# yjtang249/MIPSFusion

Hardware: NVIDIA B200
Metric: map_step_rays_per_s (higher is better)
Workload: dtype f32 (decoder contractions as bf16x3 hi/lo splits on tcgen05, fp32 accumulate; encodings, render, losses, Adam in fp32)

## Files before the change

### include/mipsfusion_b200.h

```cpp
#ifndef MIPSFUSION_B200_H
#define MIPSFUSION_B200_H

#include <stdint.h>

#ifdef __cplusplus
extern "C" {
#endif

#define MF_ABI_VERSION 2
#define MF_MAX_LEVELS 16
#define MF_MLP_PARAMS 36577
#define MF_RAW_DIM 10

#define MF_OK 0
#define MF_ERR_INVALID (-1)
#define MF_ERR_CUDA (-2)
#define MF_ERR_UNSUPPORTED (-3)

typedef struct {
    int32_t n_levels, n_features, log2_hashmap_size, base_resolution;
    float scale[MF_MAX_LEVELS];
    uint32_t resolution[MF_MAX_LEVELS];
    uint32_t size[MF_MAX_LEVELS];
    uint32_t offset[MF_MAX_LEVELS + 1];
// ... 74 lines not shown
int mf_field_query_rays_bwd(const float* rays_o, const float* rays_d, const float* z, const mf_field* field_host,
                            const float* d_raw, const void* feat, float* grad_grid, float* grad_mlp, float* d_rays_o,
                            float* d_rays_d, float* workspace, int64_t R, int S, void* stream);

int mf_render_loss_fwd(const float* raw, const float* z, const float* target_rgb, const float* target_d,
                       const int64_t* counts, const mf_render_cfg* cfg_host, float* out_rgb, float* out_depth,
                       float* out_aux, float* out_weights, int32_t* inds, float* losses, float* scratch,
                       int64_t R, int S, void* stream);
int mf_sample_z_ld(const float* target_d, int ld_d, const float* u, const float* lin_uniform, const float* lin_range,
                   const float* lin_fallback, const mf_render_cfg* cfg_host, float* z, int64_t* counts, int64_t R, void* stream);
int mf_render_loss_fwd_ld(const float* raw, const float* z, const float* target_rgb, int ld_rgb, const float* target_d, int ld_d,
                          const int64_t* counts, const mf_render_cfg* cfg_host, float* out_rgb, float* out_depth,
                          float* out_aux, float* out_weights, int32_t* inds, float* losses, float* scratch,
                          int64_t R, int S, void* stream);
int mf_render_loss_bwd(const float* raw, const float* z, const float* target_rgb, const float* target_d,
                       const int64_t* counts, const float* losses, const mf_render_cfg* cfg_host,
                       const float* g_losses, const float* g_rgb, const float* g_depth, float* d_raw,
                       int64_t R, int S, void* stream);
int mf_render_loss_bwd_scalars(const float* raw, const float* z, const float* target_rgb, int ld_rgb, const float* target_d, int ld_d,
                               const float* losses, const mf_render_cfg* cfg_host, const float* g_rgb_loss, const float* g_depth_loss,
                               const float* g_sdf_loss, const float* g_fs_loss, const float* g_rgb, const float* g_depth,
                               float* d_raw, int64_t R, int S, void* stream);

int mf_adam_step(float* p, float* g, float* m, float* v, int64_t n, double lr, double beta1, double beta2,
                 double eps, double weight_decay, int step, int zero_grad, void* stream);

int mf_adam_step_sharded(const uint64_t* peer_bases, int world, int rank, int64_t off_p, int64_t off_g, int64_t off_g_clear,
                         float* m, float* v, int64_t n, double lr, double beta1, double beta2, double eps,
                         double weight_decay, int step, uint64_t multicast_base, void* stream);
int mf_adam_step_pair(float* p0, float* g0, float* m0, float* v0, int64_t n0, double lr0, double eps0, double wd0,
                      float* p1, float* g1, float* m1, float* v1, int64_t n1, double lr1, double eps1, double wd1,
                      double beta1, double beta2, int step, void* stream);
int mf_adam_step_multi(int n_tensors, float* const* p_host, float* const* g_host, float* const* m_host,
                       float* const* v_host, const int64_t* n_host, double lr, double beta1, double beta2, double eps,
                       double weight_decay, int step, int zero_grad, void* stream);

int mf_containment(const float* dirs_cam, const float* depth, const float* pose_c2w, const float* pts, const float* xyz_min,
                   const float* xyz_max, int k, int64_t n, int cross, uint8_t* mask, int64_t* counts, void* stream);

int mf_sample_pixels_uniform(int img_h, int img_w, int num_h, int num_w, int64_t* rows, int64_t* cols, void* stream);
int64_t mf_topk_workspace_size(int64_t n);
int mf_sample_pixels_topk(const float* depth, const float* keys, int img_h, int img_w, int lattice_h, int lattice_w,
                          int num, int64_t* indices, int64_t* rows, int64_t* cols, void* workspace, void* stream);

int mf_gen_rays(const float* dirs_cam, const float* poses, const int64_t* pose_idx, float* rays_o, float* rays_d,
                int64_t R, int K, void* stream);
// ... 89 lines not shown
```

### mipsfusion_b200/_lib.py

```python
import ctypes as C
import os

import torch

_HERE = os.path.dirname(os.path.abspath(__file__))
LIB_PATH = os.environ.get("MIPSFUSION_B200_LIB") or os.path.join(_HERE, "libmipsfusion_b200.so")
HEADER_PATH = os.path.join(os.path.dirname(_HERE), "include", "mipsfusion_b200.h")

MF_MAX_LEVELS = 16
MF_MLP_PARAMS = 36577
MF_RAW_DIM = 10
MF_MAX_SAMPLES = 128


class GridMeta(C.Structure):
    _fields_ = [("n_levels", C.c_int32), ("n_features", C.c_int32), ("log2_hashmap_size", C.c_int32),
                ("base_resolution", C.c_int32), ("scale", C.c_float * MF_MAX_LEVELS),
                ("resolution", C.c_uint32 * MF_MAX_LEVELS), ("size", C.c_uint32 * MF_MAX_LEVELS),
                ("offset", C.c_uint32 * (MF_MAX_LEVELS + 1)), ("hashed", C.c_uint32 * MF_MAX_LEVELS)]


class Field(C.Structure):
    _fields_ = [("grid", C.c_void_p), ("mlp_prep", C.c_void_p), ("norm_a", C.c_double * 3), ("norm_b", C.c_double * 3),
                ("norm_factor", C.c_double), ("decoder_impl", C.c_int32), ("reserved", C.c_int32), ("meta", GridMeta)]
# ... 36 lines not shown
    "mf_debug_kernel_ms": (_I, [_I, _P]),
    "mf_hashgrid_meta": (_I, [_I, _I, _I, _I, _D, C.POINTER(GridMeta)]),
    "mf_hashgrid_fwd": (_I, [_P, _P, C.POINTER(GridMeta), _P, _P, _L, _P]),
    "mf_hashgrid_bwd": (_I, [_P, _P, _P, C.POINTER(GridMeta), _P, _P, _L, _P]),
    "mf_freq_fwd": (_I, [_P, _P, _I, _I, _L, _P]),
    "mf_freq_bwd": (_I, [_P, _P, _P, _I, _I, _L, _P]),
    "mf_mlp_prep_size": (_L, []),
    "mf_mlp_prepare": (_I, [_P, _P, _P]),
    "mf_mlp_fwd": (_I, [_P, _P, _P, _P, _P, _L, _P]),
    "mf_field_bwd_workspace_size": (_L, [_L, _I]),
    "mf_mlp_grad_workspace_size": (_L, []),
    "mf_mlp_bwd": (_I, [_P, _P, _P, _P, _P, _P, _P, _P, _P, _P, _L, _P]),
    "mf_field_query": (_I, [_P, C.POINTER(Field), _I, _P, _L, _P]),
    "mf_field_query_bwd": (_I, [_P, C.POINTER(Field), _I, _P, _P, _P, _P, _P, _L, _P]),
    "mf_sample_z": (_I, [_P, _P, _P, _P, _P, C.POINTER(RenderCfg), _P, _P, _L, _P]),
    "mf_feat_cache_size": (_L, [_L]),
    "mf_field_query_rays": (_I, [_P, _P, _P, C.POINTER(Field), _P, _P, _L, _I, _P]),
    "mf_field_query_rays_bwd": (_I, [_P, _P, _P, C.POINTER(Field), _P, _P, _P, _P, _P, _P, _P, _L, _I, _P]),
    "mf_render_loss_fwd": (_I, [_P, _P, _P, _P, _P, C.POINTER(RenderCfg), _P, _P, _P, _P, _P, _P, _P, _L, _I, _P]),
    "mf_render_loss_bwd": (_I, [_P, _P, _P, _P, _P, _P, C.POINTER(RenderCfg), _P, _P, _P, _P, _L, _I, _P]),
    "mf_render_loss_bwd_scalars": (_I, [_P, _P, _P, _I, _P, _I, _P, C.POINTER(RenderCfg), _P, _P, _P, _P, _P, _P, _P, _L, _I, _P]),
    "mf_sample_z_ld": (_I, [_P, _I, _P, _P, _P, _P, C.POINTER(RenderCfg), _P, _P, _L, _P]),
    "mf_render_loss_fwd_ld": (_I, [_P, _P, _P, _I, _P, _I, _P, C.POINTER(RenderCfg), _P, _P, _P, _P, _P, _P, _P, _L, _I, _P]),
    "mf_adam_step": (_I, [_P, _P, _P, _P, _L, _D, _D, _D, _D, _D, _I, _I, _P]),
    "mf_adam_step_sharded": (_I, [_P, _I, _I, _L, _L, _L, _P, _P, _L, _D, _D, _D, _D, _D, _I, C.c_uint64, _P]),
    "mf_adam_step_pair": (_I, [_P, _P, _P, _P, _L, _D, _D, _D, _P, _P, _P, _P, _L, _D, _D, _D, _D, _D, _I, _P]),
    "mf_adam_step_multi": (_I, [_I, _P, _P, _P, _P, _P, _D, _D, _D, _D, _D, _I, _I, _P]),
    "mf_sample_pixels_uniform": (_I, [_I, _I, _I, _I, _P, _P, _P]),
    "mf_topk_workspace_size": (_L, [_L]),
    "mf_sample_pixels_topk": (_I, [_P, _P, _I, _I, _I, _I, _I, _P, _P, _P, _P, _P]),
    "mf_gen_rays": (_I, [_P, _P, _P, _P, _P, _L, _I, _P]),
    "mf_kf_store": (_I, [_P, _P, _P, _P, _P, _I, _L, _P, _P]),
    "mf_kf_gather_rays": (_I, [_P, _L, _L, _P, _L, _I, _P, _L, _P, _L, _P, _L, _P, _P, _P, _P]),
    "mf_sample_distinct": (_I, [_L, _L, C.c_uint32, _P, _P]),
    "mf_kf_sample_rays": (_I, [_P, _L, _L, _P, _L, _L, _I, _L, _L, _L, C.c_uint32, _P, _P, _P, _P, _P]),
    "mf_frame_sample_rays": (_I, [_P, _P, _P, _I, _I, _L, C.c_uint32, _P, _P, _P, _P]),
    "mf_gen_rays_packed": (_I, [_P, _P, _P, _P, _P, _P, _P, _L, _I, _P]),
    "mf_gen_rays_bwd": (_I, [_P, _P, _P, _P, _P, _L, _I, _P]),
    "mf_gen_rays_packed_bwd": (_I, [_P, _P, _P, _P, _P, _L, _I, _P]),
    "mf_pose_to_c2w": (_I, [_P, _P, _P]),
    "mf_pose_refine_update": (_I, [_P, _P, _P, _P, _P, _D, _D, _I, _P, _P]),
    "mf_track_handoff": (_I, [_P, _P, _P, _P, _P]),
    "mf_ba_pose_init": (_I, [_P, _P, _I, _P, _P, _P]),
    "mf_ba_pose_update": (_I, [_P, _P, _P, _I, _D, _D, _P, _P]),
    "mf_ro_score": (_I, [_P, _P, _P, _P, _P, _P, C.POINTER(Field), _D, _D, _I, _I, _I, _P, _P, _P, _P, _P]),
    "mf_ro_update": (_I, [_P, _P, _P, _I, _D, _P, _P, _P, _P, _P, _P]),
# ... 77 lines not shown
```

### mipsfusion_b200/csrc/field_kernels.cu

```cuda
#include "field_bwd.cuh"
#include "field_launch.cuh"
#include "field_tc_launch.cuh"
#include "field_tc_bwd.cuh"
#include "field_tc_bwd2.cuh"
#include "field_tc_bwd3.cuh"

__device__ __forceinline__ void mlp_prepare_simt(const float* __restrict__ mlp, float* __restrict__ prep, int i) {
    if (i >= PREP_SIMT_SIZE) return;
    float v = 0.f;
    if (i < MF_MLP_PARAMS) {
        v = mlp[i];
    } else if (i >= PREP_F1) {
        int r;
        if (i < PREP_B1) {
            int off, K, Kreal;
            if (i < PREP_F2) { r = i - PREP_F1; off = OFF_W1; K = D_E; Kreal = D_E; }
            else if (i < PREP_F3) { r = i - PREP_F2; off = OFF_W2; K = D_H; Kreal = D_H; }
            else { r = i - PREP_F3; off = OFF_WS1; K = D_SDF_IN; Kreal = D_SDF_IN; }
            const int k = r >> 7, tx = (r >> 3) & 15, i8 = r & 7;
            const int n = tx + 16 * i8;
            v = (k < Kreal) ? mlp[off + n * K + k] : 0.f;
        } else {
            int off, K, KI;
            if (i < PREP_B2) { r = i - PREP_B1; off = OFF_W1; K = D_E; KI = 4; }
// ... 487 lines not shown
    if (N >= (int64_t)1 << 31) { mf_set_error("backward: more than 2^31 points"); return MF_ERR_INVALID; }
    const int64_t nb = act_blocks(N);
    int* idx = reinterpret_cast<int*>(scratch);
    uint32_t* flags = reinterpret_cast<uint32_t*>(idx + N);
    int* blk_cnt = reinterpret_cast<int*>(flags + nb * 32);
    int* count = blk_cnt + nb;
    active_count_kernel<<<(unsigned)nb, ACT_BLK, 0, st>>>(d_raw, N, flags, blk_cnt);
    MF_LAUNCH_CHECK();
    active_fill_kernel<<<(unsigned)nb, ACT_BLK, 0, st>>>(flags, blk_cnt, idx, count);
    MF_LAUNCH_CHECK();
    am->idx = idx; am->count = count;
    return MF_OK;
}

static inline int64_t cta_scratch_words() { return (int64_t)mf_sm_count_cached() * b2::SCR_CTA_WORDS; }

MF_API int64_t mf_field_bwd_workspace_size(int64_t n_points, int want_point_grads) {
    if (n_points < 0) n_points = 0;
    return mf_mlp_grad_workspace_size() + (want_point_grads ? 3 * n_points : 0) + act_scratch_words(n_points) + cta_scratch_words();
}

template <class Src>
static int launch_field_bwd(const FieldDev& d, const Src& src, const float* d_raw, float* grad_grid, float* grad_mlp,
                            float* d_pts, float* workspace, float* scratch, int64_t N, cudaStream_t st) {
    ActiveMap am{nullptr, nullptr};
    int rc0 = compact_active_points(d_raw, N, scratch, &am, st); if (rc0) return rc0;
    if (d_pts) MF_CUDA(cudaMemsetAsync(d_pts, 0, (size_t)N * 3 * sizeof(float), st));
    const bool params = grad_grid != nullptr;
    if (!params && !d_pts) {
        mf_set_error("backward without parameter gradients needs a ray / point gradient output");
        return MF_ERR_INVALID;
    }
    if (!params && d.impl == 1) {
        const int grid = persistent_grid(N, 1);
        int rc = set_smem(field_bwd_dx_kernel<Src>, SMEM_BWD); if (rc) return rc;
        field_bwd_dx_kernel<Src><<<grid, NT, SMEM_BWD, st>>>(d, src, d_raw, d_pts, N, am);
        MF_LAUNCH_CHECK();
        return MF_OK;
    }
    if (d.impl != 1) {
        const int64_t tiles = (N + TC_TP - 1) / TC_TP;
        const int64_t cap = mf_sm_count_cached();
        const int grid = (int)(tiles < cap ? (tiles > 0 ? tiles : 1) : cap);
        mf_ktimer_begin(1, st);
        if (!params) {
            int rc = set_smem(field_bwd_tc_kernel<Src, true, false>, SMEM_TC_BWD); if (rc) return rc;
            field_bwd_tc_kernel<Src, true, false><<<grid, TC_NT, SMEM_TC_BWD, st>>>(d, src, d_raw, nullptr, nullptr, d_pts, N, am, mf_tc_error_flag(), mf_tc_profile_buffer());
            mf_ktimer_end(1, st);
            MF_LAUNCH_CHECK();
// ... 83 lines not shown
MF_API int mf_field_query_rays_bwd(const float* rays_o, const float* rays_d, const float* z, const mf_field* field,
                                   const float* d_raw, const void* feat, float* grad_grid, float* grad_mlp, float* d_rays_o,
                                   float* d_rays_d, float* workspace, int64_t R, int S, void* stream) {
    MF_CHECK_ARG(R >= 0 && S > 0);
    if (R == 0) return MF_OK;
    MF_CHECK_ARG(rays_o && rays_d && z && d_raw && workspace);
    MF_CHECK_ARG((grad_grid == nullptr) == (grad_mlp == nullptr));
    MF_CHECK_ARG(((uintptr_t)grad_grid & 15) == 0);
    MF_CHECK_ARG((d_rays_o == nullptr) == (d_rays_d == nullptr));
    FieldDev d; int rc = mf_field_to_dev(field, &d); if (rc) return rc;
    d.feat = (uint32_t*)feat;
    SrcRays src{rays_o, rays_d, z, S};
    cudaStream_t st = (cudaStream_t)stream;
    float* d_pts = d_rays_o ? workspace + mf_mlp_grad_workspace_size() : nullptr;
    float* scratch = workspace + mf_mlp_grad_workspace_size() + (d_rays_o ? 3 * R * S : 0);
    rc = launch_field_bwd(d, src, d_raw, grad_grid, grad_mlp, d_pts, workspace, scratch, R * S, st);
    if (rc) return rc;
    if (d_rays_o) {
        ray_grad_reduce_kernel<<<(unsigned)((R + 7) / 8), 256, 0, st>>>(d_pts, z, d_rays_o, d_rays_d, R, S);
        MF_LAUNCH_CHECK();
    }
    return MF_OK;
}
```

### mipsfusion_b200/csrc/render_kernels.cu

```cuda
#include <limits.h>

#include "mf_common.cuh"

constexpr int MAX_S = 128;

struct RenderCfgDev {
    int n_u, n_r, perturb, rgb_missing_nz;
    float tr;
    float sctr;
    float T;
    float twoT;
    float depth_trunc;
    float emd_w;
    int ld_rgb, ld_d;
};

static RenderCfgDev cfg_to_dev(const mf_render_cfg* c) {
    RenderCfgDev d;
    d.n_u = c->n_samples_d; d.n_r = c->n_range_d; d.perturb = c->perturb; d.rgb_missing_nz = c->rgb_missing_nz;
    d.tr = (float)c->trunc; d.sctr = (float)(c->sc_factor * c->trunc);
    const double T = c->trunc * c->sc_factor;
    d.T = (float)T; d.twoT = (float)(2.0 * T);
    d.depth_trunc = (float)c->depth_trunc; d.emd_w = (float)c->emd_w;
    d.ld_rgb = 3; d.ld_d = 1;
    return d;
}

__global__ void sample_z_kernel(const float* __restrict__ target_d, const float* __restrict__ u,
                                const float* __restrict__ lin_u, const float* __restrict__ lin_r,
                                const float* __restrict__ lin_fb, RenderCfgDev c, float* __restrict__ z,
                                unsigned long long* __restrict__ counts, int64_t R) {
    extern __shared__ float zs[];
    __shared__ int cnt[2];
    const int64_t r = blockIdx.x;
    const int S = c.n_u + c.n_r;
    const bool has_d = target_d != nullptr;
    const float d = has_d ? target_d[r * c.ld_d] : 0.f;
    const bool around = d > 0.f;
    if (threadIdx.x < 2) cnt[threadIdx.x] = 0;
    for (int e = threadIdx.x; e < S; e += blockDim.x) {
        float v; int rank;
        if (e < c.n_u) {
            v = lin_u[e]; rank = e;
            for (int k = 0; k < c.n_r; ++k) {
                const float sv = around ? __fadd_rn(lin_r[k], d) : lin_fb[k];
                rank += (sv < v);
            }
        } else {
            const int k = e - c.n_u;
            v = around ? __fadd_rn(lin_r[k], d) : lin_fb[k];
            rank = k;
            for (int i = 0; i < c.n_u; ++i) rank += (lin_u[i] <= v);
        }
        zs[rank] = v;
    }
    __syncthreads();
    int n_front = 0, n_sdf = 0;
    for (int j = threadIdx.x; j < S; j += blockDim.x) {
        float zj = zs[j];
        if (c.perturb && u) {
            const float lower = (j == 0) ? zs[0] : 0.5f * __fadd_rn(zs[j], zs[j - 1]);
            const float upper = (j == S - 1) ? zs[S - 1] : 0.5f * __fadd_rn(zs[j + 1], zs[j]);
// ... 121 lines not shown
        sdf2 = fmaf(e2, e2, sdf2);
        if (c.emd_w > 0.f) {
            const float* p = raw + (r * S + s) * MF_RAW_DIM + 5;
            const float gt = __fdiv_rn(__fadd_rn(__fsub_rn(d, zz), c.T), c.twoT) * 4.0f;
            float a = 0.f, b = 0.f;
#pragma unroll
            for (int k = 0; k < 5; ++k) { a = fmaf(p[k], (float)(4 - k), a); b = fmaf(fabsf(gt - (float)k), p[k], b); }
            fs1 = fmaf(a, fm, fs1);
            sdf1 = fmaf(b, sm_, sdf1);
        }
    }
    fs2 = warp_sum(fs2); sdf2 = warp_sum(sdf2); fs1 = warp_sum(fs1); sdf1 = warp_sum(sdf1);
    if (lane == 0) {
        float rs = 0.f;
        if (target_rgb)
#pragma unroll
            for (int k = 0; k < 3; ++k) { const float e = rgb[k] * mk - target_rgb[r * c.ld_rgb + k] * mk; rs = fmaf(e, e, rs); }
        float* sc = scratch + r * 8;
        sc[0] = rs; sc[1] = valid ? (depth - d) * (depth - d) : 0.f; sc[2] = valid ? 1.f : 0.f;
        sc[3] = fs2; sc[4] = sdf2; sc[5] = fs1; sc[6] = sdf1; sc[7] = 0.f;
    }
}

__global__ void __launch_bounds__(1024) loss_finalize_kernel(const float* __restrict__ scratch,
                                                             const unsigned long long* __restrict__ counts,
                                                             RenderCfgDev c, float* __restrict__ losses, int64_t R, int S) {
    __shared__ double red[32][8];
    double s[8] = {0, 0, 0, 0, 0, 0, 0, 0};
    const float4* rows = reinterpret_cast<const float4*>(scratch);
    for (int64_t r = threadIdx.x; r < R; r += 1024) {
        const float4 a = rows[2 * r], b = rows[2 * r + 1];
        s[0] += (double)a.x; s[1] += (double)a.y; s[2] += (double)a.z; s[3] += (double)a.w;
        s[4] += (double)b.x; s[5] += (double)b.y; s[6] += (double)b.z;
    }
#pragma unroll
    for (int k = 0; k < 7; ++k) s[k] = warp_sum_d(s[k]);
    const int w = threadIdx.x >> 5, lane = threadIdx.x & 31;
    if (lane == 0)
#pragma unroll
        for (int k = 0; k < 7; ++k) red[w][k] = s[k];
    __syncthreads();
    if (w != 0) return;
    double t[7];
#pragma unroll
    for (int k = 0; k < 7; ++k) t[k] = warp_sum_d(red[lane][k]);
    if (threadIdx.x == 0) {
        const double RS = (double)R * (double)S;
        const float n_fs = (float)counts[0], n_sdf = (float)counts[1];
        const float n = (float)(counts[0] + counts[1]);
        const float fs_w = 1.0f - n_fs / n, sdf_w = 1.0f - n_sdf / n;
        const float rgb_loss = (float)(t[0] / (3.0 * (double)R));
        const float depth_loss = (float)(t[1] / t[2]);
        float fs_loss = (float)(t[3] / RS) * fs_w, sdf_loss = (float)(t[4] / RS) * sdf_w;
        if (c.emd_w > 0.f) {
            fs_loss += (float)(t[5] / RS) / 250.0f * c.emd_w;
            sdf_loss += (float)(t[6] / RS) / 5000.0f * c.emd_w;
        }
        losses[0] = rgb_loss; losses[1] = depth_loss; losses[2] = sdf_loss; losses[3] = fs_loss;
        losses[4] = -10.0f * logf(rgb_loss) / logf(10.0f);
        losses[5] = fs_w; losses[6] = sdf_w; losses[7] = (float)t[2];
    }
}

struct LossGrads { const float* p[4]; };

__global__ void __launch_bounds__(256) render_loss_bwd_kernel(
    const float* __restrict__ raw, const float* __restrict__ z, const float* __restrict__ target_rgb,
    const float* __restrict__ target_d, const float* __restrict__ losses, RenderCfgDev c,
    LossGrads g_losses, const float* __restrict__ g_rgb, const float* __restrict__ g_depth,
    float* __restrict__ d_raw, int64_t R, int S) {
    const int64_t r = (int64_t)blockIdx.x * 8 + (threadIdx.x >> 5);
    const int lane = threadIdx.x & 31;
    if (r >= R) return;
// ... 53 lines not shown
            const bool back = zz > __fadd_rn(d, c.T);
            const float fm = front ? 1.f : 0.f;
            const float sm_ = (!front && !back && d > 0.f) ? 1.f : 0.f;
            dsdf += gl_fs * fs_w * 2.0f * (sd * fm - fm) * fm * invRS;
            dsdf += gl_sdf * sdf_w * 2.0f * ((zz + sd * c.T) * sm_ - d * sm_) * sm_ * c.T * invRS;
            if (c.emd_w > 0.f) {
                const float gt = __fdiv_rn(__fadd_rn(__fsub_rn(d, zz), c.T), c.twoT) * 4.0f;
#pragma unroll
                for (int k = 0; k < 5; ++k)
                    dp[k] = gl_fs * c.emd_w * fm * (float)(4 - k) * invRS / 250.0f +
                            gl_sdf * c.emd_w * sm_ * fabsf(gt - (float)k) * invRS / 5000.0f;
            }
        }
        const float w = q.wt[t] * inv;
        float orgb[3];
#pragma unroll
        for (int k = 0; k < 3; ++k) orgb[k] = G_rgb[k] * w * sg[t][k] * (1.0f - sg[t][k]);
        float2* o2 = reinterpret_cast<float2*>(o);
        o2[0] = make_float2(orgb[0], orgb[1]); o2[1] = make_float2(orgb[2], dsdf); o2[2] = make_float2(0.f, dp[0]);
        o2[3] = make_float2(dp[1], dp[2]); o2[4] = make_float2(dp[3], dp[4]);
    }
}

__global__ void gen_rays_kernel(const float* __restrict__ dirs, int ld, const float* __restrict__ poses,
                                const int64_t* __restrict__ pose_idx, float* __restrict__ rays_o,
                                float* __restrict__ rays_d, float* __restrict__ rgb, float* __restrict__ depth, int64_t R, int K) {
    const int64_t r = (int64_t)blockIdx.x * blockDim.x + threadIdx.x;
    if (r >= R) return;
    int64_t pi = pose_idx ? pose_idx[r] : 0;
    if (pi < 0) pi += K;
    const float* P = poses + pi * 16;
    const float dx = dirs[r * ld], dy = dirs[r * ld + 1], dz = dirs[r * ld + 2];
    if (rgb) { rgb[r * 3] = dirs[r * ld + 3]; rgb[r * 3 + 1] = dirs[r * ld + 4]; rgb[r * 3 + 2] = dirs[r * ld + 5]; }
    if (depth) depth[r] = dirs[r * ld + 6];
#pragma unroll
    for (int j = 0; j < 3; ++j) {
        rays_d[r * 3 + j] = __fadd_rn(__fadd_rn(__fmul_rn(dx, P[j * 4]), __fmul_rn(dy, P[j * 4 + 1])), __fmul_rn(dz, P[j * 4 + 2]));
        rays_o[r * 3 + j] = P[j * 4 + 3];
    }
}

constexpr int GRB_MAX_K = 64;
__global__ void __launch_bounds__(256) gen_rays_bwd_kernel(const float* __restrict__ dirs, int dir_stride, const int64_t* __restrict__ pose_idx,
                                                           const float* __restrict__ d_o, const float* __restrict__ d_d,
                                                           float* __restrict__ d_poses, int64_t R, int K) {
    __shared__ float acc[GRB_MAX_K * 12];
// ... 16 lines not shown
                atomicAdd(&acc[pi * 12 + j * 4 + 3], d_o[r * 3 + j]);
            } else {
                float* P = d_poses + pi * 16;
#pragma unroll
                for (int k = 0; k < 3; ++k) atomicAdd(&P[j * 4 + k], g * dv[k]);
                atomicAdd(&P[j * 4 + 3], d_o[r * 3 + j]);
            }
        }
    }
    if (use_smem) {
        __syncthreads();
        for (int i = threadIdx.x; i < K * 12; i += blockDim.x) {
            const float v = acc[i];
            if (v != 0.f) atomicAdd(&d_poses[(i / 12) * 16 + (i % 12)], v);
        }
    }
}

MF_API int mf_sample_z(const float* target_d, const float* u, const float* lin_uniform, const float* lin_range,
                       const float* lin_fallback, const mf_render_cfg* cfg, float* z, int64_t* counts, int64_t R, void* stream) {
    return mf_sample_z_ld(target_d, 1, u, lin_uniform, lin_range, lin_fallback, cfg, z, counts, R, stream);
}

MF_API int mf_sample_z_ld(const float* target_d, int ld_d, const float* u, const float* lin_uniform, const float* lin_range,
                          const float* lin_fallback, const mf_render_cfg* cfg, float* z, int64_t* counts, int64_t R, void* stream) {
    MF_CHECK_ARG(cfg && z && R >= 0 && ld_d >= 1);
    if (R == 0) return MF_OK;
    RenderCfgDev c = cfg_to_dev(cfg);
    c.ld_d = ld_d;
    if (!target_d) c.n_r = 0;
    const int S = c.n_u + c.n_r;
    MF_CHECK_ARG(S > 0 && S <= 4096);
    MF_CHECK_ARG(c.n_u == 0 || lin_uniform);
    MF_CHECK_ARG(c.n_r == 0 || (lin_range && lin_fallback));
    MF_CHECK_ARG(!target_d || counts);
    cudaStream_t st = (cudaStream_t)stream;
    if (counts) MF_CUDA(cudaMemsetAsync(counts, 0, 2 * sizeof(int64_t), st));
    const int threads = S <= 32 ? 32 : (S <= 64 ? 64 : 128);
    sample_z_kernel<<<(unsigned)R, threads, S * sizeof(float), st>>>(target_d, u, lin_uniform, lin_range, lin_fallback, c, z,
                                                                      (unsigned long long*)counts, R);
    MF_LAUNCH_CHECK();
    return MF_OK;
}

MF_API int mf_render_loss_fwd(const float* raw, const float* z, const float* target_rgb, const float* target_d,
                              const int64_t* counts, const mf_render_cfg* cfg, float* out_rgb, float* out_depth,
                              float* out_aux, float* out_weights, int32_t* inds, float* losses, float* scratch, int64_t R, int S,
                              void* stream) {
    return mf_render_loss_fwd_ld(raw, z, target_rgb, 3, target_d, 1, counts, cfg, out_rgb, out_depth, out_aux, out_weights, inds, losses,
                                 scratch, R, S, stream);
}

MF_API int mf_render_loss_fwd_ld(const float* raw, const float* z, const float* target_rgb, int ld_rgb, const float* target_d, int ld_d,
                                 const int64_t* counts, const mf_render_cfg* cfg, float* out_rgb, float* out_depth,
                                 float* out_aux, float* out_weights, int32_t* inds, float* losses, float* scratch, int64_t R, int S,
                                 void* stream) {
    MF_CHECK_ARG(cfg && raw && z && out_rgb && out_depth && R >= 0 && ld_rgb >= 3 && ld_d >= 1);
    MF_CHECK_ARG(S > 0 && S <= MAX_S);
    if (R == 0) return MF_OK;
    MF_CHECK_ARG(!target_d || (counts && losses && scratch));
    RenderCfgDev c = cfg_to_dev(cfg);
    c.ld_rgb = ld_rgb; c.ld_d = ld_d;
    cudaStream_t st = (cudaStream_t)stream;
// ... 87 lines not shown
```

### mipsfusion_b200/mapper.py

```python
import ctypes as C

import torch

from . import _lib as L
from . import dist as D
from .decoder import _Workspace
from .keyframe_store import _new_seed, frame_tensors


class FusedMapper:
    def __init__(self, model, lr_decoder=None, lr_embed=None, group=None, peer_memory="auto", multicast="auto"):
        self.model = model
        cfg = model.config
        self.dev = model._device
        if self.dev.type != "cuda":
            raise L.MipsFusionB200Error("FusedMapper needs the model on a CUDA device")
        self.lr_decoder = cfg["mapping"]["lr_decoder"] if lr_decoder is None else lr_decoder
        self.lr_embed = cfg["mapping"]["lr_embed"] if lr_embed is None else lr_embed
        self.group = group
        self.world = D.world(group)[0]
        t = cfg["training"]
        self.loss_w = torch.tensor([t["rgb_weight"], t["depth_weight"], t["sdf_weight"], t["fs_weight"]], dtype=torch.float32,
                                   device=self.dev)
        self.grid = model.embed_fn.params.data
# ... 1 lines not shown
        self._mlp_pad = torch.zeros((nm + 3) // 4 * 4, device=self.dev, dtype=torch.float32)
        self._mlp_pad[:nm].copy_(model.decoder.flat_weights())
        self.mlp = self._mlp_pad[:nm]
        self.prep = torch.empty(int(L.lib().mf_mlp_prep_size()), device=self.dev, dtype=torch.float32)
        self.g_grid = torch.zeros_like(self.grid); self.m_grid = torch.zeros_like(self.grid); self.v_grid = torch.zeros_like(self.grid)
        self._g_mlp_pad = torch.zeros_like(self._mlp_pad); self.g_mlp = self._g_mlp_pad[:nm]
        self.m_mlp = torch.zeros_like(self._mlp_pad); self.v_mlp = torch.zeros_like(self._mlp_pad)
        self.arena = None
        self.multicast = multicast
        if self.world > 1 and peer_memory:
            try:
                self._init_peer_arena()
            except Exception as e:
                if peer_memory is True:
                    raise
                import warnings
                warnings.warn("FusedMapper: peer memory unavailable (%s); using NCCL all-reduce" % (e,))
                self.arena = None
        if self.world > 1 and self.dev.type == "cuda":
            L.call("mf_set_sm_reserve", 1)
        self.step_count = 0
        self.pose_grad_impl = "tc"
        self._bufs = {}
        self.timing = None
        self.launches = 0
        with torch.cuda.device(self.dev):
            L.call("mf_mlp_prepare", L.ptr(self.mlp), L.ptr(self.prep), L.stream())
        self._bind_module()

    def _bind_module(self):
        dec, o = self.model.decoder, 0
        ps = dec.ordered_params()
        with torch.no_grad():
            for p in ps:
                n = p.numel()
                p.data = self.mlp[o:o + n].view(p.shape)
                o += n
        self._seen_versions = tuple(p._version for p in ps)
        dec.__dict__.pop("_prep_cache", None)
        dec.__dict__["_ext_prep"] = (tuple(p.data_ptr() for p in ps), self)

    def _init_peer_arena(self):
        ng, nm = self.grid.numel(), self.mlp.numel()
        arena = D.PeerArena({"p_grid": ng, "g_grid0": ng, "g_grid1": ng, "p_mlp": nm, "g_mlp0": nm, "g_mlp1": nm}, self.dev, self.group)
        arena.view("p_grid", ng).copy_(self.grid)
        arena.view("p_mlp", nm).copy_(self.mlp)
        self.grid = arena.view("p_grid", ng)
        self.model.embed_fn.params.data = self.grid
        self.mlp = arena.view("p_mlp", nm)
        self._g_grid = [arena.view("g_grid0", ng), arena.view("g_grid1", ng)]
        self._g_mlp = [arena.view("g_mlp0", nm), arena.view("g_mlp1", nm)]
        self.g_grid, self.g_mlp = self._g_grid[0], self._g_mlp[0]
        nm4 = arena.sizes["p_mlp"]
        self.m_mlp = torch.zeros(nm4, device=self.dev); self.v_mlp = torch.zeros(nm4, device=self.dev)
        self.arena = arena
        torch.cuda.current_stream(self.dev).synchronize()
        arena.barrier()

    def _buffers(self, R, S):
        key = (R, S)
        b = self._bufs.get(key)
        if b is None:
            d = self.dev
            f32 = dict(device=d, dtype=torch.float32)
            b = dict(z=torch.empty(R, S, **f32), counts=torch.empty(2, device=d, dtype=torch.int64),
                     raw=torch.empty(R, S, L.MF_RAW_DIM, **f32), d_raw=torch.empty(R, S, L.MF_RAW_DIM, **f32),
                     rgb=torch.empty(R, 3, **f32), depth=torch.empty(R, **f32), losses=torch.zeros(8, **f32),
                     scratch=torch.empty(R * 8, **f32), u=torch.empty(R, S, **f32),
                     feat=torch.empty(int(L.lib().mf_feat_cache_size(R * S)), device=d, dtype=torch.uint8))
            self._bufs[key] = b
        return b

    def _field(self):
        f = self.model._field(keep=(self.grid, self.prep))
        return f

    def step(self, rays_o, rays_d, target_rgb, target_d, u=None, EMD_w=0.01, update=True, ray_grads=None):
        model = self.model
        R = rays_o.shape[0]
        cfg, lins = model._render_cfg(True, EMD_w, self.dev)
        S = cfg.n_samples_d + cfg.n_range_d
        b = self._buffers(R, S)
        st = L.stream()
        field = self._field()
        target_d = target_d.reshape(R)
        if cfg.perturb:
            if u is None:
                u = b["u"].uniform_()
        else:
            u = None
        tm = self.timing
        def ev():
            if tm is None:
                return None
            e = torch.cuda.Event(enable_timing=True); e.record(); return e
        e0 = ev()
        L.call("mf_sample_z", L.ptr(target_d), L.ptr(u), L.ptr(lins[0]), L.ptr(lins[1]), L.ptr(lins[2]), C.byref(cfg),
               L.ptr(b["z"]), L.ptr(b["counts"]), R, st)
        work = D.allreduce_sum_async_(b["counts"], self.group)
        e1 = ev()
        L.call("mf_field_query_rays", L.ptr(rays_o), L.ptr(rays_d), L.ptr(b["z"]), C.byref(field), L.ptr(b["raw"]), L.ptr(b["feat"]),
               R, S, st)
        if work is not None:
            work.wait()
        e2 = ev()
        L.call("mf_render_loss_fwd", L.ptr(b["raw"]), L.ptr(b["z"]), L.ptr(target_rgb), L.ptr(target_d), L.ptr(b["counts"]),
               C.byref(cfg), L.ptr(b["rgb"]), L.ptr(b["depth"]), None, None, None, L.ptr(b["losses"]), L.ptr(b["scratch"]), R, S, st)
        L.call("mf_render_loss_bwd", L.ptr(b["raw"]), L.ptr(b["z"]), L.ptr(target_rgb), L.ptr(target_d), L.ptr(b["counts"]),
               L.ptr(b["losses"]), C.byref(cfg), L.ptr(self.loss_w), None, None, L.ptr(b["d_raw"]), R, S, st)
        e3 = ev()
        if ray_grads is None:
            L.call("mf_field_query_rays_bwd", L.ptr(rays_o), L.ptr(rays_d), L.ptr(b["z"]), C.byref(field), L.ptr(b["d_raw"]),
                   L.ptr(b["feat"]), L.ptr(self.g_grid), L.ptr(self.g_mlp), None, None, L.ptr(_Workspace.get(self.dev, field_points=R * S)), R, S, st)
        else:
            fb = field if self.pose_grad_impl == "tc" else self.model._field(keep=(self.grid, self.prep), impl=1)
            L.call("mf_field_query_rays_bwd", L.ptr(rays_o), L.ptr(rays_d), L.ptr(b["z"]), C.byref(fb), L.ptr(b["d_raw"]),
                   L.ptr(b["feat"]) if self.pose_grad_impl == "tc" else None, L.ptr(self.g_grid), L.ptr(self.g_mlp), L.ptr(ray_grads[0]), L.ptr(ray_grads[1]),
                   L.ptr(_Workspace.get(self.dev, field_points=R * S, want_ray_grads=True)), R, S, st)
            self.launches += 2
        e4 = ev()
        self.launches += 9
        if update:
            if self.arena is not None:
                self.apply_gradients_sharded()
            else:
                D.average_gradients_([self.g_grid, self.g_mlp], self.group)
                self.apply_gradients()
        e5 = ev()
        if tm is not None:
            for name, a, c in (("sample_z", e0, e1), ("field_fwd", e1, e2), ("render_loss", e2, e3), ("field_bwd", e3, e4),
                               ("adam", e4, e5)):
                tm.setdefault(name, []).append((a, c))
        return b["losses"]

    def step_host(self, rays7, pose_idx, poses, EMD_w=0.01, pose_grad=False):
        R = rays7.shape[0]
        hb = self._bufs.get(("host", R))
        if hb is None:
            f32 = dict(device=self.dev, dtype=torch.float32)
            hb = dict(rays7=torch.empty(R, 7, **f32), idx=torch.empty(R, device=self.dev, dtype=torch.int64),
                      o=torch.empty(R, 3, **f32), d=torch.empty(R, 3, **f32), rgb=torch.empty(R, 3, **f32),
                      depth=torch.empty(R, **f32), out=torch.empty(8, dtype=torch.float32).pin_memory())
            self._bufs[("host", R)] = hb
        hb["rays7"].copy_(rays7, non_blocking=True)
# ... 252 lines not shown
```

Measured before the change: 7.208 million.

## Fuse render loss forward/backward with active-point compaction for mapping step

Adds a single render_loss_map kernel that computes rendered color/depth, per-ray loss partials and d_raw in one pass. The sample_z kernel now also counts valid-depth rays, so the gradient can be formed without waiting for the finalized losses. The kernel also builds the compacted active-sample index list with a decoupled look-back prefix scan, so the field backward skips its own compaction pass. Loss finalization moves to a side stream that overlaps the field backward. In exchange the code relies on a single-pass look-back scan with spin-waiting on block status, and it adds a separate code path that runs only when no pose gradients are requested.

```diff
diff --git a/include/mipsfusion_b200.h b/include/mipsfusion_b200.h
--- a/include/mipsfusion_b200.h
+++ b/include/mipsfusion_b200.h
@@ -120,6 +120,18 @@
                                const float* g_sdf_loss, const float* g_fs_loss, const float* g_rgb, const float* g_depth,
                                float* d_raw, int64_t R, int S, void* stream);
 
+int64_t mf_map_state_size(int64_t R);
+int mf_sample_z_map(const float* target_d, const float* u, const float* lin_uniform, const float* lin_range,
+                    const float* lin_fallback, const mf_render_cfg* cfg_host, float* z, int64_t* state, int64_t R, void* stream);
+int mf_render_loss_map(const float* raw, const float* z, const float* target_rgb, const float* target_d, int64_t* state,
+                       const mf_render_cfg* cfg_host, const float* loss_w, float* out_rgb, float* out_depth, float* scratch,
+                       float* d_raw, int32_t* act, int64_t R, int S, void* stream);
+int mf_loss_finalize(const float* scratch, const int64_t* counts, const mf_render_cfg* cfg_host, float* losses, int64_t R, int S,
+                     void* stream);
+int mf_field_query_rays_bwd_act(const float* rays_o, const float* rays_d, const float* z, const mf_field* field_host,
+                                const float* d_raw, const void* feat, const int32_t* act, float* grad_grid, float* grad_mlp,
+                                float* workspace, int64_t R, int S, void* stream);
+
 int mf_adam_step(float* p, float* g, float* m, float* v, int64_t n, double lr, double beta1, double beta2,
                  double eps, double weight_decay, int step, int zero_grad, void* stream);
 
diff --git a/mipsfusion_b200/_lib.py b/mipsfusion_b200/_lib.py
--- a/mipsfusion_b200/_lib.py
+++ b/mipsfusion_b200/_lib.py
@@ -82,6 +82,11 @@
     "mf_render_loss_bwd_scalars": (_I, [_P, _P, _P, _I, _P, _I, _P, C.POINTER(RenderCfg), _P, _P, _P, _P, _P, _P, _P, _L, _I, _P]),
     "mf_sample_z_ld": (_I, [_P, _I, _P, _P, _P, _P, C.POINTER(RenderCfg), _P, _P, _L, _P]),
     "mf_render_loss_fwd_ld": (_I, [_P, _P, _P, _I, _P, _I, _P, C.POINTER(RenderCfg), _P, _P, _P, _P, _P, _P, _P, _L, _I, _P]),
+    "mf_map_state_size": (_L, [_L]),
+    "mf_sample_z_map": (_I, [_P, _P, _P, _P, _P, C.POINTER(RenderCfg), _P, _P, _L, _P]),
+    "mf_render_loss_map": (_I, [_P, _P, _P, _P, _P, C.POINTER(RenderCfg), _P, _P, _P, _P, _P, _P, _L, _I, _P]),
+    "mf_loss_finalize": (_I, [_P, _P, C.POINTER(RenderCfg), _P, _L, _I, _P]),
+    "mf_field_query_rays_bwd_act": (_I, [_P, _P, _P, C.POINTER(Field), _P, _P, _P, _P, _P, _P, _L, _I, _P]),
     "mf_adam_step": (_I, [_P, _P, _P, _P, _L, _D, _D, _D, _D, _D, _I, _I, _P]),
     "mf_adam_step_sharded": (_I, [_P, _I, _I, _L, _L, _L, _P, _P, _L, _D, _D, _D, _D, _D, _I, C.c_uint64, _P]),
     "mf_adam_step_pair": (_I, [_P, _P, _P, _P, _L, _D, _D, _D, _P, _P, _P, _P, _L, _D, _D, _D, _D, _D, _I, _P]),
diff --git a/mipsfusion_b200/csrc/field_kernels.cu b/mipsfusion_b200/csrc/field_kernels.cu
--- a/mipsfusion_b200/csrc/field_kernels.cu
+++ b/mipsfusion_b200/csrc/field_kernels.cu
@@ -533,9 +533,10 @@
 
 template <class Src>
 static int launch_field_bwd(const FieldDev& d, const Src& src, const float* d_raw, float* grad_grid, float* grad_mlp,
-                            float* d_pts, float* workspace, float* scratch, int64_t N, cudaStream_t st) {
+                            float* d_pts, float* workspace, float* scratch, int64_t N, cudaStream_t st, const ActiveMap* pre = nullptr) {
     ActiveMap am{nullptr, nullptr};
-    int rc0 = compact_active_points(d_raw, N, scratch, &am, st); if (rc0) return rc0;
+    if (pre) am = *pre;
+    else { int rc0 = compact_active_points(d_raw, N, scratch, &am, st); if (rc0) return rc0; }
     if (d_pts) MF_CUDA(cudaMemsetAsync(d_pts, 0, (size_t)N * 3 * sizeof(float), st));
     const bool params = grad_grid != nullptr;
     if (!params && !d_pts) {
@@ -665,3 +666,19 @@
     }
     return MF_OK;
 }
+
+MF_API int mf_field_query_rays_bwd_act(const float* rays_o, const float* rays_d, const float* z, const mf_field* field,
+                                       const float* d_raw, const void* feat, const int32_t* act, float* grad_grid, float* grad_mlp,
+                                       float* workspace, int64_t R, int S, void* stream) {
+    MF_CHECK_ARG(R >= 0 && S > 0);
+    if (R == 0) return MF_OK;
+    MF_CHECK_ARG(rays_o && rays_d && z && d_raw && act && grad_grid && grad_mlp && workspace);
+    MF_CHECK_ARG(((uintptr_t)grad_grid & 15) == 0);
+    MF_CHECK_ARG(R * S < ((int64_t)1 << 31));
+    FieldDev d; int rc = mf_field_to_dev(field, &d); if (rc) return rc;
+    d.feat = (uint32_t*)feat;
+    SrcRays src{rays_o, rays_d, z, S};
+    const ActiveMap am{act, act + R * S};
+    return launch_field_bwd(d, src, d_raw, grad_grid, grad_mlp, nullptr, workspace, workspace + mf_mlp_grad_workspace_size(), R * S,
+                            (cudaStream_t)stream, &am);
+}
diff --git a/mipsfusion_b200/csrc/render_kernels.cu b/mipsfusion_b200/csrc/render_kernels.cu
--- a/mipsfusion_b200/csrc/render_kernels.cu
+++ b/mipsfusion_b200/csrc/render_kernels.cu
@@ -29,7 +29,7 @@
 __global__ void sample_z_kernel(const float* __restrict__ target_d, const float* __restrict__ u,
                                 const float* __restrict__ lin_u, const float* __restrict__ lin_r,
                                 const float* __restrict__ lin_fb, RenderCfgDev c, float* __restrict__ z,
-                                unsigned long long* __restrict__ counts, int64_t R) {
+                                unsigned long long* __restrict__ counts, unsigned long long* __restrict__ n_valid, int64_t R) {
     extern __shared__ float zs[];
     __shared__ int cnt[2];
     const int64_t r = blockIdx.x;
@@ -38,6 +38,7 @@
     const float d = has_d ? target_d[r * c.ld_d] : 0.f;
     const bool around = d > 0.f;
     if (threadIdx.x < 2) cnt[threadIdx.x] = 0;
+    if (n_valid && threadIdx.x == 0 && d > 0.f && d < c.depth_trunc) atomicAdd(n_valid, 1ull);
     for (int e = threadIdx.x; e < S; e += blockDim.x) {
         float v; int rank;
         if (e < c.n_u) {
@@ -205,6 +206,12 @@
     }
 }
 
+__device__ __forceinline__ void mask_weights(const unsigned long long* __restrict__ counts, float& fs_w, float& sdf_w) {
+    const float n_fs = (float)counts[0], n_sdf = (float)counts[1];
+    const float n = (float)(counts[0] + counts[1]);
+    fs_w = 1.0f - n_fs / n; sdf_w = 1.0f - n_sdf / n;
+}
+
 __global__ void __launch_bounds__(1024) loss_finalize_kernel(const float* __restrict__ scratch,
                                                              const unsigned long long* __restrict__ counts,
                                                              RenderCfgDev c, float* __restrict__ losses, int64_t R, int S) {
@@ -229,9 +236,8 @@
     for (int k = 0; k < 7; ++k) t[k] = warp_sum_d(red[lane][k]);
     if (threadIdx.x == 0) {
         const double RS = (double)R * (double)S;
-        const float n_fs = (float)counts[0], n_sdf = (float)counts[1];
-        const float n = (float)(counts[0] + counts[1]);
-        const float fs_w = 1.0f - n_fs / n, sdf_w = 1.0f - n_sdf / n;
+        float fs_w, sdf_w;
+        mask_weights(counts, fs_w, sdf_w);
         const float rgb_loss = (float)(t[0] / (3.0 * (double)R));
         const float depth_loss = (float)(t[1] / t[2]);
         float fs_loss = (float)(t[3] / RS) * fs_w, sdf_loss = (float)(t[4] / RS) * sdf_w;
@@ -331,6 +337,188 @@
     }
 }
 
+constexpr int MAP_RAYS = 8;
+static inline int64_t map_blocks(int64_t R) { return (R + MAP_RAYS - 1) / MAP_RAYS; }
+constexpr unsigned long long LB_AGG = 1ull << 32, LB_INC = 2ull << 32;
+
+__device__ __forceinline__ unsigned long long lb_load(const unsigned long long* p) { return *reinterpret_cast<const volatile unsigned long long*>(p); }
+__device__ __forceinline__ void lb_store(unsigned long long* p, unsigned long long v) { *reinterpret_cast<volatile unsigned long long*>(p) = v; }
+
+__global__ void __launch_bounds__(256) render_loss_map_kernel(
+    const float* __restrict__ raw, const float* __restrict__ z, const float* __restrict__ target_rgb,
+    const float* __restrict__ target_d, unsigned long long* __restrict__ state, RenderCfgDev c, const float* __restrict__ loss_w,
+    float* __restrict__ out_rgb, float* __restrict__ out_depth, float* __restrict__ scratch, float* __restrict__ d_raw,
+    int* __restrict__ act_idx, int* __restrict__ act_count, int64_t R, int S) {
+    __shared__ int s_blk, s_base, s_warp[MAP_RAYS];
+    if (threadIdx.x == 0) s_blk = (int)atomicAdd(&state[3], 1ull);
+    __syncthreads();
+    const int64_t blk = s_blk;
+    const int warp = threadIdx.x >> 5, lane = threadIdx.x & 31;
+    const int64_t r = blk * MAP_RAYS + warp;
+    uint32_t ball[4] = {0u, 0u, 0u, 0u};
+    if (r < R) {
+        float sg[4][3];
+#pragma unroll
+        for (int t = 0; t < 4; ++t) {
+            const int s = lane + 32 * t;
+#pragma unroll
+            for (int k = 0; k < 3; ++k) sg[t][k] = s < S ? raw[(r * S + s) * MF_RAW_DIM + k] : 0.f;
+        }
+        RaySamples q;
+        load_ray(raw, z, r, S, lane, c, q);
+        const float inv = 1.0f / (q.wsum + 1e-8f);
+        float rgb[3] = {0.f, 0.f, 0.f}, depth = 0.f;
+#pragma unroll
+        for (int t = 0; t < 4; ++t) {
+            const float w = q.wt[t] * inv;
+#pragma unroll
+            for (int k = 0; k < 3; ++k) {
+                sg[t][k] = q.in[t] ? sigmoidf_(sg[t][k]) : 0.f;
+                rgb[k] = fmaf(w, sg[t][k], rgb[k]);
+            }
+            depth = fmaf(w, q.z[t], depth);
+        }
+#pragma unroll
+        for (int k = 0; k < 3; ++k) rgb[k] = warp_sum(rgb[k]);
+        depth = warp_sum(depth);
+        const float d = target_d[r * c.ld_d];
+        const bool valid = d > 0.f && d < c.depth_trunc;
+        const float mk = (valid || c.rgb_missing_nz) ? 1.f : 0.f;
+        float fs2 = 0.f, sdf2 = 0.f, fs1 = 0.f, sdf1 = 0.f;
+#pragma unroll
+        for (int t = 0; t < 4; ++t) {
+            if (!q.in[t]) continue;
+            const int s = lane + 32 * t;
+            const float zz = q.z[t], sd = q.sdf[t];
+            const bool front = zz < __fsub_rn(d, c.T);
+            const bool back = zz > __fadd_rn(d, c.T);
+            const float fm = front ? 1.f : 0.f;
+            const float sm_ = (!front && !back && d > 0.f) ? 1.f : 0.f;
+            const float e1 = sd * fm - fm;
+            fs2 = fmaf(e1, e1, fs2);
+            const float e2 = (zz + sd * c.T) * sm_ - d * sm_;
+            sdf2 = fmaf(e2, e2, sdf2);
+            if (c.emd_w > 0.f) {
+                const float* p = raw + (r * S + s) * MF_RAW_DIM + 5;
+                const float gt = __fdiv_rn(__fadd_rn(__fsub_rn(d, zz), c.T), c.twoT) * 4.0f;
+                float a = 0.f, b = 0.f;
+#pragma unroll
+                for (int k = 0; k < 5; ++k) { a = fmaf(p[k], (float)(4 - k), a); b = fmaf(fabsf(gt - (float)k), p[k], b); }
+                fs1 = fmaf(a, fm, fs1);
+                sdf1 = fmaf(b, sm_, sdf1);
+            }
+        }
+        fs2 = warp_sum(fs2); sdf2 = warp_sum(sdf2); fs1 = warp_sum(fs1); sdf1 = warp_sum(sdf1);
+        if (lane == 0) {
+            out_rgb[r * 3] = rgb[0]; out_rgb[r * 3 + 1] = rgb[1]; out_rgb[r * 3 + 2] = rgb[2];
+            out_depth[r] = depth;
+            float rs = 0.f;
+            if (target_rgb)
+#pragma unroll
+                for (int k = 0; k < 3; ++k) { const float e = rgb[k] * mk - target_rgb[r * c.ld_rgb + k] * mk; rs = fmaf(e, e, rs); }
+            float* sc = scratch + r * 8;
+            sc[0] = rs; sc[1] = valid ? (depth - d) * (depth - d) : 0.f; sc[2] = valid ? 1.f : 0.f;
+            sc[3] = fs2; sc[4] = sdf2; sc[5] = fs1; sc[6] = sdf1; sc[7] = 0.f;
+        }
+        float fs_w, sdf_w;
+        mask_weights(state, fs_w, sdf_w);
+        const float n_valid = (float)state[2];
+        const float gl_rgb = __ldg(loss_w), gl_depth = __ldg(loss_w + 1), gl_sdf = __ldg(loss_w + 2), gl_fs = __ldg(loss_w + 3);
+        float G_rgb[3], G_depth = 0.f;
+#pragma unroll
+        for (int k = 0; k < 3; ++k) {
+            G_rgb[k] = 0.f;
+            if (target_rgb) G_rgb[k] += gl_rgb * 2.0f * mk * (rgb[k] * mk - target_rgb[r * c.ld_rgb + k] * mk) / (3.0f * (float)R);
+        }
+        if (valid && gl_depth != 0.f) G_depth += gl_depth * 2.0f * (depth - d) / n_valid;
+        float a[4], abar = 0.f;
+#pragma unroll
+        for (int t = 0; t < 4; ++t) {
+            a[t] = G_rgb[0] * sg[t][0] + G_rgb[1] * sg[t][1] + G_rgb[2] * sg[t][2] + G_depth * q.z[t];
+            abar = fmaf(q.wt[t] * inv, a[t], abar);
+        }
+        abar = warp_sum(abar);
+        const float invRS = 1.0f / ((float)R * (float)S);
+#pragma unroll
+        for (int t = 0; t < 4; ++t) {
+            bool on = false;
+            if (q.in[t]) {
+                const int s = lane + 32 * t;
+                const float zz = q.z[t], sd = q.sdf[t], sgm = q.sig[t];
+                float* o = d_raw + (r * S + s) * MF_RAW_DIM;
+                float dsdf = 0.f;
+                if (q.wt[t] != 0.f) dsdf = (a[t] - abar) * inv * (sgm * (1.0f - sgm) * (1.0f - 2.0f * sgm)) / c.tr;
+                float dp[5] = {0.f, 0.f, 0.f, 0.f, 0.f};
+                const bool front = zz < __fsub_rn(d, c.T);
+                const bool back = zz > __fadd_rn(d, c.T);
+                const float fm = front ? 1.f : 0.f;
+                const float sm_ = (!front && !back && d > 0.f) ? 1.f : 0.f;
+                dsdf += gl_fs * fs_w * 2.0f * (sd * fm - fm) * fm * invRS;
+                dsdf += gl_sdf * sdf_w * 2.0f * ((zz + sd * c.T) * sm_ - d * sm_) * sm_ * c.T * invRS;
+                if (c.emd_w > 0.f) {
+                    const float gt = __fdiv_rn(__fadd_rn(__fsub_rn(d, zz), c.T), c.twoT) * 4.0f;
+#pragma unroll
+                    for (int k = 0; k < 5; ++k)
+                        dp[k] = gl_fs * c.emd_w * fm * (float)(4 - k) * invRS / 250.0f +
+                                gl_sdf * c.emd_w * sm_ * fabsf(gt - (float)k) * invRS / 5000.0f;
+                }
+                const float w = q.wt[t] * inv;
+                float orgb[3];
+#pragma unroll
+                for (int k = 0; k < 3; ++k) orgb[k] = G_rgb[k] * w * sg[t][k] * (1.0f - sg[t][k]);
+                float2* o2 = reinterpret_cast<float2*>(o);
+                o2[0] = make_float2(orgb[0], orgb[1]); o2[1] = make_float2(orgb[2], dsdf); o2[2] = make_float2(0.f, dp[0]);
+                o2[3] = make_float2(dp[1], dp[2]); o2[4] = make_float2(dp[3], dp[4]);
+                on = (orgb[0] != 0.f) | (orgb[1] != 0.f) | (orgb[2] != 0.f) | (dsdf != 0.f) | (dp[0] != 0.f) | (dp[1] != 0.f) |
+                     (dp[2] != 0.f) | (dp[3] != 0.f) | (dp[4] != 0.f);
+            }
+            ball[t] = __ballot_sync(0xffffffffu, on);
+        }
+    }
+    if (lane == 0) s_warp[warp] = __popc(ball[0]) + __popc(ball[1]) + __popc(ball[2]) + __popc(ball[3]);
+    __syncthreads();
+    if (warp == 0) {
+        const int own = lane < MAP_RAYS ? s_warp[lane] : 0;
+        int v = own;
+#pragma unroll
+        for (int o = 1; o < 32; o <<= 1) { const int t = __shfl_up_sync(0xffffffffu, v, o); if (lane >= o) v += t; }
+        const int agg = __shfl_sync(0xffffffffu, v, MAP_RAYS - 1);
+        if (lane < MAP_RAYS) s_warp[lane] = v - own;
+        unsigned long long* status = state + 4;
+        int prefix = 0;
+        if (blk == 0) {
+            if (lane == 0) lb_store(&status[0], LB_INC | (unsigned)agg);
+        } else {
+            if (lane == 0) lb_store(&status[blk], LB_AGG | (unsigned)agg);
+            for (int64_t j = blk - 1;; j -= 32) {
+                const int64_t jj = j - lane;
+                unsigned long long w = jj >= 0 ? lb_load(&status[jj]) : LB_INC;
+                while (__any_sync(0xffffffffu, (w >> 32) == 0))
+                    if ((w >> 32) == 0) w = lb_load(&status[jj]);
+                const uint32_t inc = __ballot_sync(0xffffffffu, (w >> 32) == 2);
+                const int first = inc ? __ffs(inc) - 1 : 31;
+                prefix += __reduce_add_sync(0xffffffffu, lane <= first ? (unsigned)(uint32_t)w : 0u);
+                if (inc) break;
+            }
+            if (lane == 0) lb_store(&status[blk], LB_INC | (unsigned)(prefix + agg));
+        }
+        if (lane == 0) {
+            s_base = prefix;
+            if (blk == (int64_t)gridDim.x - 1) *act_count = prefix + agg;
+        }
+    }
+    __syncthreads();
+    if (r < R) {
+        int pos = s_base + s_warp[warp];
+        const uint32_t lt = (1u << lane) - 1u;
+#pragma unroll
+        for (int t = 0; t < 4; ++t) {
+            if ((ball[t] >> lane) & 1u) act_idx[pos + __popc(ball[t] & lt)] = (int)(r * S + lane + 32 * t);
+            pos += __popc(ball[t]);
+        }
+    }
+}
+
 __global__ void gen_rays_kernel(const float* __restrict__ dirs, int ld, const float* __restrict__ poses,
                                 const int64_t* __restrict__ pose_idx, float* __restrict__ rays_o,
                                 float* __restrict__ rays_d, float* __restrict__ rgb, float* __restrict__ depth, int64_t R, int K) {
@@ -393,8 +581,9 @@
     return mf_sample_z_ld(target_d, 1, u, lin_uniform, lin_range, lin_fallback, cfg, z, counts, R, stream);
 }
 
-MF_API int mf_sample_z_ld(const float* target_d, int ld_d, const float* u, const float* lin_uniform, const float* lin_range,
-                          const float* lin_fallback, const mf_render_cfg* cfg, float* z, int64_t* counts, int64_t R, void* stream) {
+static int sample_z_launch(const float* target_d, int ld_d, const float* u, const float* lin_uniform, const float* lin_range,
+                           const float* lin_fallback, const mf_render_cfg* cfg, float* z, int64_t* counts, int64_t n_clear, int64_t R,
+                           void* stream) {
     MF_CHECK_ARG(cfg && z && R >= 0 && ld_d >= 1);
     if (R == 0) return MF_OK;
     RenderCfgDev c = cfg_to_dev(cfg);
@@ -406,10 +595,47 @@
     MF_CHECK_ARG(c.n_r == 0 || (lin_range && lin_fallback));
     MF_CHECK_ARG(!target_d || counts);
     cudaStream_t st = (cudaStream_t)stream;
-    if (counts) MF_CUDA(cudaMemsetAsync(counts, 0, 2 * sizeof(int64_t), st));
+    if (counts) MF_CUDA(cudaMemsetAsync(counts, 0, n_clear * sizeof(int64_t), st));
     const int threads = S <= 32 ? 32 : (S <= 64 ? 64 : 128);
     sample_z_kernel<<<(unsigned)R, threads, S * sizeof(float), st>>>(target_d, u, lin_uniform, lin_range, lin_fallback, c, z,
-                                                                      (unsigned long long*)counts, R);
+                                                                      (unsigned long long*)counts,
+                                                                      n_clear > 2 ? (unsigned long long*)counts + 2 : nullptr, R);
+    MF_LAUNCH_CHECK();
+    return MF_OK;
+}
+
+MF_API int mf_sample_z_ld(const float* target_d, int ld_d, const float* u, const float* lin_uniform, const float* lin_range,
+                          const float* lin_fallback, const mf_render_cfg* cfg, float* z, int64_t* counts, int64_t R, void* stream) {
+    return sample_z_launch(target_d, ld_d, u, lin_uniform, lin_range, lin_fallback, cfg, z, counts, 2, R, stream);
+}
+
+MF_API int64_t mf_map_state_size(int64_t R) { return 4 + map_blocks(R < 0 ? 0 : R); }
+
+MF_API int mf_sample_z_map(const float* target_d, const float* u, const float* lin_uniform, const float* lin_range, const float* lin_fallback,
+                           const mf_render_cfg* cfg, float* z, int64_t* state, int64_t R, void* stream) {
+    MF_CHECK_ARG(target_d && state);
+    return sample_z_launch(target_d, 1, u, lin_uniform, lin_range, lin_fallback, cfg, z, state, mf_map_state_size(R), R, stream);
+}
+
+MF_API int mf_render_loss_map(const float* raw, const float* z, const float* target_rgb, const float* target_d, int64_t* state,
+                              const mf_render_cfg* cfg, const float* loss_w, float* out_rgb, float* out_depth, float* scratch,
+                              float* d_raw, int32_t* act, int64_t R, int S, void* stream) {
+    MF_CHECK_ARG(cfg && raw && z && target_d && state && loss_w && out_rgb && out_depth && scratch && d_raw && act && R >= 0);
+    MF_CHECK_ARG(S > 0 && S <= MAX_S && ((uintptr_t)d_raw & 7) == 0);
+    MF_CHECK_ARG(R * S < ((int64_t)1 << 31));
+    if (R == 0) return MF_OK;
+    const RenderCfgDev c = cfg_to_dev(cfg);
+    render_loss_map_kernel<<<(unsigned)map_blocks(R), MAP_RAYS * 32, 0, (cudaStream_t)stream>>>(
+        raw, z, target_rgb, target_d, (unsigned long long*)state, c, loss_w, out_rgb, out_depth, scratch, d_raw, act, act + R * S, R, S);
+    MF_LAUNCH_CHECK();
+    return MF_OK;
+}
+
+MF_API int mf_loss_finalize(const float* scratch, const int64_t* counts, const mf_render_cfg* cfg, float* losses, int64_t R, int S,
+                            void* stream) {
+    MF_CHECK_ARG(scratch && counts && cfg && losses && R >= 0 && S > 0);
+    if (R == 0) return MF_OK;
+    loss_finalize_kernel<<<1, 1024, 0, (cudaStream_t)stream>>>(scratch, (const unsigned long long*)counts, cfg_to_dev(cfg), losses, R, S);
     MF_LAUNCH_CHECK();
     return MF_OK;
 }
diff --git a/mipsfusion_b200/mapper.py b/mipsfusion_b200/mapper.py
--- a/mipsfusion_b200/mapper.py
+++ b/mipsfusion_b200/mapper.py
@@ -47,6 +47,7 @@
         self.step_count = 0
         self.pose_grad_impl = "tc"
         self._bufs = {}
+        self._side = None
         self.timing = None
         self.launches = 0
         with torch.cuda.device(self.dev):
@@ -88,13 +89,20 @@
         if b is None:
             d = self.dev
             f32 = dict(device=d, dtype=torch.float32)
-            b = dict(z=torch.empty(R, S, **f32), counts=torch.empty(2, device=d, dtype=torch.int64),
+            state = torch.empty(int(L.lib().mf_map_state_size(R)), device=d, dtype=torch.int64)
+            b = dict(z=torch.empty(R, S, **f32), state=state, counts=state[:2], act=torch.empty(R * S + 1, device=d, dtype=torch.int32),
                      raw=torch.empty(R, S, L.MF_RAW_DIM, **f32), d_raw=torch.empty(R, S, L.MF_RAW_DIM, **f32),
                      rgb=torch.empty(R, 3, **f32), depth=torch.empty(R, **f32), losses=torch.zeros(8, **f32),
                      scratch=torch.empty(R * 8, **f32), u=torch.empty(R, S, **f32),
                      feat=torch.empty(int(L.lib().mf_feat_cache_size(R * S)), device=d, dtype=torch.uint8))
             self._bufs[key] = b
         return b
+
+    def _side_stream(self):
+        if self._side is None:
+            self._side = torch.cuda.Stream(self.dev)
+            self._ev_fork, self._ev_join = torch.cuda.Event(), torch.cuda.Event()
+        return self._side
 
     def _field(self):
         f = self.model._field(keep=(self.grid, self.prep))
@@ -119,9 +127,14 @@
             if tm is None:
                 return None
             e = torch.cuda.Event(enable_timing=True); e.record(); return e
+        fused = ray_grads is None
         e0 = ev()
-        L.call("mf_sample_z", L.ptr(target_d), L.ptr(u), L.ptr(lins[0]), L.ptr(lins[1]), L.ptr(lins[2]), C.byref(cfg),
-               L.ptr(b["z"]), L.ptr(b["counts"]), R, st)
+        if fused:
+            L.call("mf_sample_z_map", L.ptr(target_d), L.ptr(u), L.ptr(lins[0]), L.ptr(lins[1]), L.ptr(lins[2]), C.byref(cfg),
+                   L.ptr(b["z"]), L.ptr(b["state"]), R, st)
+        else:
+            L.call("mf_sample_z", L.ptr(target_d), L.ptr(u), L.ptr(lins[0]), L.ptr(lins[1]), L.ptr(lins[2]), C.byref(cfg),
+                   L.ptr(b["z"]), L.ptr(b["counts"]), R, st)
         work = D.allreduce_sum_async_(b["counts"], self.group)
         e1 = ev()
         L.call("mf_field_query_rays", L.ptr(rays_o), L.ptr(rays_d), L.ptr(b["z"]), C.byref(field), L.ptr(b["raw"]), L.ptr(b["feat"]),
@@ -129,22 +142,35 @@
         if work is not None:
             work.wait()
         e2 = ev()
-        L.call("mf_render_loss_fwd", L.ptr(b["raw"]), L.ptr(b["z"]), L.ptr(target_rgb), L.ptr(target_d), L.ptr(b["counts"]),
-               C.byref(cfg), L.ptr(b["rgb"]), L.ptr(b["depth"]), None, None, None, L.ptr(b["losses"]), L.ptr(b["scratch"]), R, S, st)
-        L.call("mf_render_loss_bwd", L.ptr(b["raw"]), L.ptr(b["z"]), L.ptr(target_rgb), L.ptr(target_d), L.ptr(b["counts"]),
-               L.ptr(b["losses"]), C.byref(cfg), L.ptr(self.loss_w), None, None, L.ptr(b["d_raw"]), R, S, st)
+        if fused:
+            L.call("mf_render_loss_map", L.ptr(b["raw"]), L.ptr(b["z"]), L.ptr(target_rgb), L.ptr(target_d), L.ptr(b["state"]),
+                   C.byref(cfg), L.ptr(self.loss_w), L.ptr(b["rgb"]), L.ptr(b["depth"]), L.ptr(b["scratch"]), L.ptr(b["d_raw"]),
+                   L.ptr(b["act"]), R, S, st)
+            side = self._side_stream()
+            self._ev_fork.record(torch.cuda.current_stream(self.dev))
+            side.wait_event(self._ev_fork)
+            L.call("mf_loss_finalize", L.ptr(b["scratch"]), L.ptr(b["counts"]), C.byref(cfg), L.ptr(b["losses"]), R, S, side.cuda_stream)
+        else:
+            L.call("mf_render_loss_fwd", L.ptr(b["raw"]), L.ptr(b["z"]), L.ptr(target_rgb), L.ptr(target_d), L.ptr(b["counts"]),
+                   C.byref(cfg), L.ptr(b["rgb"]), L.ptr(b["depth"]), None, None, None, L.ptr(b["losses"]), L.ptr(b["scratch"]), R, S, st)
+            L.call("mf_render_loss_bwd", L.ptr(b["raw"]), L.ptr(b["z"]), L.ptr(target_rgb), L.ptr(target_d), L.ptr(b["counts"]),
+                   L.ptr(b["losses"]), C.byref(cfg), L.ptr(self.loss_w), None, None, L.ptr(b["d_raw"]), R, S, st)
         e3 = ev()
-        if ray_grads is None:
-            L.call("mf_field_query_rays_bwd", L.ptr(rays_o), L.ptr(rays_d), L.ptr(b["z"]), C.byref(field), L.ptr(b["d_raw"]),
-                   L.ptr(b["feat"]), L.ptr(self.g_grid), L.ptr(self.g_mlp), None, None, L.ptr(_Workspace.get(self.dev, field_points=R * S)), R, S, st)
+        if fused:
+            L.call("mf_field_query_rays_bwd_act", L.ptr(rays_o), L.ptr(rays_d), L.ptr(b["z"]), C.byref(field), L.ptr(b["d_raw"]),
+                   L.ptr(b["feat"]), L.ptr(b["act"]), L.ptr(self.g_grid), L.ptr(self.g_mlp),
+                   L.ptr(_Workspace.get(self.dev, field_points=R * S)), R, S, st)
+            self._ev_join.record(side)
+            torch.cuda.current_stream(self.dev).wait_event(self._ev_join)
+            self.launches += 6
         else:
             fb = field if self.pose_grad_impl == "tc" else self.model._field(keep=(self.grid, self.prep), impl=1)
             L.call("mf_field_query_rays_bwd", L.ptr(rays_o), L.ptr(rays_d), L.ptr(b["z"]), C.byref(fb), L.ptr(b["d_raw"]),
                    L.ptr(b["feat"]) if self.pose_grad_impl == "tc" else None, L.ptr(self.g_grid), L.ptr(self.g_mlp), L.ptr(ray_grads[0]), L.ptr(ray_grads[1]),
                    L.ptr(_Workspace.get(self.dev, field_points=R * S, want_ray_grads=True)), R, S, st)
             self.launches += 2
+            self.launches += 9
         e4 = ev()
-        self.launches += 9
         if update:
             if self.arena is not None:
                 self.apply_gradients_sharded()
```

After: 7.515 million (median of 6 runs). 1.04x the previous value.
